# CFSAN-Biostatistics/snp-pipeline

Hardware: AMD Instinct MI355X
Metric: consensus_bases_called_per_sec (higher is better)
Workload: dtype u8; 1 GPU; BASELINE configs[3] shard (125 samples/GPU x 5000000 bp x 30x synthetic pileups, 49878 SNP sites, 1500 SNP records per sample; the reference bundles no pileups); step = site-record gather + site union, one batched scan launch + one call launch, 4-bit pack, row all-gather, all-pairs distance tiles, row-band exchange; samples_total=125, samples_this_rank=125, genome_bp=5000000, snp_sites=49878, pileup_bytes_this_rank=54061520755, parallelism=samples sharded over 1 rank(s)

## Files before the change

### include/snpgpu.h

```cpp
#ifndef SNPGPU_H
#define SNPGPU_H

#include <stddef.h>
#include <stdint.h>

#ifdef __cplusplus
extern "C" {
#endif

#define SNPGPU_ABI_VERSION 7

#define SNPGPU_OK            0
#define SNPGPU_E_HIP        -1
#define SNPGPU_E_ARG        -2
#define SNPGPU_E_NOMEM      -3
#define SNPGPU_E_PILEUP     -4
#define SNPGPU_E_UNSUPPORTED -5
#define SNPGPU_E_IO         -6
#define SNPGPU_E_TIMEOUT    -7

#define SNPGPU_F_RAWDPTH  0x01
#define SNPGPU_F_VARFREQ  0x02
#define SNPGPU_F_DEPTH    0x04
#define SNPGPU_F_STRDPTH  0x08
// ... 282 lines not shown
uint32_t snpgpu_symbol_spill_capacity(const snpgpu_ctx *ctx);

typedef struct snpgpu_consensus_job {
    const char *fasta_path;
    const char *fasta_id;
    const uint8_t *sequence;
    uint64_t n_bases;
    const char *vcf_path;
    const char *vcf_header;
    const snpgpu_site_counts *counts;
    const uint64_t *line_off;
    const uint8_t *row_filters;
    const uint8_t *site_in_flow;
    int32_t rc;
    uint32_t n_rows;
} snpgpu_consensus_job;
int  snpgpu_write_consensus_files(snpgpu_consensus_job *jobs, uint32_t n_jobs, uint32_t n_sites, const uint8_t *contig_names,
                                  const uint32_t *contig_name_off, const uint64_t *site_keys, const char *const *filter_names,
                                  int preserve_ref_case, char failed_snp_gt, const snpgpu_symbol_spill *spill, uint32_t n_spill,
                                  uint32_t n_threads);

int  snpgpu_region_flow_dev(snpgpu_ctx *ctx, const uint8_t *d_base, const uint8_t *d_filters, const uint64_t *d_line_off,
                            uint32_t n_samples, uint32_t n_sites, const uint32_t *d_cols, const int32_t *d_col_of, uint32_t n_cols,
                            const uint32_t *d_excl_off, const uint32_t *d_excl_slots, uint8_t *d_out_base, uint8_t *d_out_filters,
                            uint32_t *d_err);

int  snpgpu_rows_copy_dev(snpgpu_ctx *ctx, const void *d_src, uint64_t src_stride, const uint32_t *d_src_index,
                          void *d_dst, uint64_t dst_stride, const uint32_t *d_dst_index, uint32_t n_rows, uint64_t row_bytes);

int  snpgpu_siteset_line_offsets(snpgpu_ctx *ctx, const snpgpu_siteset *ss, uint64_t *out_line_off);

#define SNPGPU_CALL_PASSES 4
int  snpgpu_call_pass_counts(snpgpu_ctx *ctx, uint64_t out[SNPGPU_CALL_PASSES]);

size_t snpgpu_packed_row_bytes(uint32_t n_sites);
int  snpgpu_pack_matrix_dev(snpgpu_ctx *ctx, const uint8_t *d_symbols, uint32_t n_rows, uint32_t n_sites,
                            size_t row_stride, void *d_packed);
int  snpgpu_distance_packed_dev(snpgpu_ctx *ctx, const void *d_packed, uint32_t n_rows, uint32_t n_sites,
                                uint32_t tile_rank, uint32_t tile_nranks, int32_t *d_out);
int  snpgpu_distance(snpgpu_ctx *ctx, const uint8_t *symbols, uint32_t n_rows, uint32_t n_sites, int32_t *out);

int  snpgpu_vcf_sites(const char *path, uint64_t capacity, uint32_t *out_pos, uint32_t *out_contig, uint64_t *out_n_records,
                      char *out_names, uint64_t names_capacity, uint64_t *out_name_off, uint32_t names_max,
                      uint32_t *out_n_names);
int  snpgpu_snplist_sites(const char *path, uint64_t capacity, uint32_t *out_pos, uint32_t *out_contig, uint64_t *out_n_records,
                          char *out_names, uint64_t names_capacity, uint64_t *out_name_off, uint32_t names_max,
                          uint32_t *out_n_names);
int  snpgpu_write_snplist(const char *path, const char *contig_names, const uint64_t *contig_off, const uint64_t *keys,
                          uint64_t n_sites, const uint32_t *carrier_off, const uint32_t *carriers, const char *sample_names,
                          const uint64_t *sample_off);

int  snpgpu_fasta_scan(const char *path, uint64_t *out_n_records, uint64_t *out_max_len, uint64_t *out_names_bytes);
int  snpgpu_fasta_load(const char *path, uint64_t n_records, uint64_t row_stride, uint8_t pad, uint8_t *out_matrix,
                       uint64_t *out_len, char *out_names, uint64_t *out_name_off);

#define SNPGPU_TSV_PAIRWISE 0
#define SNPGPU_TSV_MATRIX   1
int  snpgpu_write_distance_tsv(const char *path, int layout, const char *ids, const uint64_t *id_off, uint32_t n,
                               const int32_t *matrix, uint64_t row_stride);

#define SNPGPU_COMM_ID_BYTES 128
int  snpgpu_comm_available(void);
int  snpgpu_comm_version(int *out_version);
int  snpgpu_comm_unique_id(void *out_id);
int  snpgpu_comm_init(snpgpu_ctx *ctx, int rank, int nranks, const void *unique_id);
void snpgpu_comm_destroy(snpgpu_ctx *ctx);
// ... 108 lines not shown
```

### snp_pipeline_amd/_lib.py

```python
import ctypes as C
import os

_HERE = os.path.dirname(os.path.abspath(__file__))
LIB_PATH = os.path.join(_HERE, "lib", "libsnpgpu.so")

MAX_SYMS = 8
SCAN_STATUS_WORDS = 4
CALL_PASSES = 4

F_RAWDPTH, F_VARFREQ, F_DEPTH, F_STRDPTH, F_STRBIAS, F_REGION = 1, 2, 4, 8, 16, 32
SITE_IN_SNPLIST, SITE_EXCLUDED = 1, 2
ST_NO_LINE, ST_OK, ST_SHORT_LINE, ST_BAD_DEPTH, ST_NO_QUALS, ST_MULTI_REF = 0, 1, 2, 3, 4, 5
VCF_LINE_WINDOW, VCF_MORE_UNUSUAL, VCF_LONG_LINE = 4096, 1, 2
E_HIP, E_ARG, E_NOMEM, E_PILEUP, E_UNSUPPORTED, E_IO, E_TIMEOUT = -1, -2, -3, -4, -5, -6, -7


class CallerParams(C.Structure):
    _fields_ = [("min_base_quality", C.c_int32), ("min_cons_depth", C.c_int32),
                ("min_cons_strand_depth", C.c_int32), ("reserved", C.c_int32),
                ("min_cons_freq", C.c_double), ("min_cons_strand_bias", C.c_double)]


class SiteCounts(C.Structure):
    _fields_ = [("raw_depth", C.c_uint32), ("good_depth", C.c_uint32), ("fwd_good_depth", C.c_uint32),
# ... 121 lines not shown
    "snpgpu_call_consensus_batch_dev": (C.c_int, [_P, _P, _P, _P, _P, C.c_uint32, C.POINTER(CallerParams), _P, _P, _P]),
    "snpgpu_call_consensus": (C.c_int, [_P, _P, _P, C.c_size_t, C.POINTER(CallerParams), _P, _P, _P, _P, C.c_int]),
    "snpgpu_call_consensus_files": (C.c_int, [_P, _P, C.POINTER(C.c_char_p), C.c_uint32, C.POINTER(CallerParams), _P, _P, _P, _P,
                                              _P, _P, _P, _P, C.POINTER(StreamOpts), C.POINTER(StreamStats)]),
    "snpgpu_call_consensus_files_dev": (C.c_int, [_P, _P, C.POINTER(C.c_char_p), C.c_uint32, C.POINTER(CallerParams), _P, _P, _P, _P,
                                                  _P, _P, _P, _P, C.POINTER(StreamOpts), C.POINTER(StreamStats)]),
    "snpgpu_call_consensus_many_dev": (C.c_int, [_P, _P, _P, _P, C.c_uint32, C.POINTER(CallerParams), _P, _P, _P, _P, _P, _P, C.c_int]),
    "snpgpu_region_flow_dev": (C.c_int, [_P, _P, _P, _P, C.c_uint32, C.c_uint32, _P, _P, C.c_uint32, _P, _P, _P, _P, _P]),
    "snpgpu_rows_copy_dev": (C.c_int, [_P, _P, C.c_uint64, _P, _P, C.c_uint64, _P, C.c_uint32, C.c_uint64]),
    "snpgpu_write_consensus_files": (C.c_int, [_P, C.c_uint32, C.c_uint32, _P, _P, _P, C.POINTER(C.c_char_p), C.c_int, C.c_char, _P, C.c_uint32,
                                               C.c_uint32]),
    "snpgpu_varscan_dev": (C.c_int, [_P, _P, C.c_uint64, _P, C.c_uint32, _P, C.POINTER(C.c_uint32), _P]),
    "snpgpu_varscan_batch_dev": (C.c_int, [_P, _P, _P, C.c_uint32, _P, C.c_uint32, _P, _P, _P, _P]),
    "snpgpu_pileups_create": (C.c_int, [_P, C.c_uint64, C.POINTER(_P)]),
    "snpgpu_pileups_destroy": (None, [_P]),
    "snpgpu_pileups_ingest": (C.c_int, [_P, _P, C.POINTER(C.c_char_p), C.c_uint32, _P, C.c_uint32, _P, _P, _P, _P, _P]),
    "snpgpu_pileups_count": (C.c_uint32, [_P]),
    "snpgpu_pileups_get": (C.c_int, [_P, C.c_uint32, C.POINTER(_P), C.POINTER(C.c_uint64)]),
    "snpgpu_pileups_get_stats": (C.c_int, [_P, C.POINTER(PileupsStats)]),
    "snpgpu_call_all_lines_file": (C.c_int, [_P, _P, C.c_char_p, C.POINTER(CallerParams), C.c_uint64, C.POINTER(C.c_uint64),
                                             _P, _P, _P, _P]),
    "snpgpu_call_all_lines_compact_file": (C.c_int, [_P, _P, C.c_char_p, C.POINTER(CallerParams), C.c_uint64, C.POINTER(C.c_uint64), _P, _P,
                                                     C.c_uint32, C.POINTER(C.c_uint32), _P, _P, _P]),
    "snpgpu_format_line_rows": (C.c_size_t, [_P, C.c_uint64, _P, _P, C.c_uint64, _P, _P, C.c_uint32, C.POINTER(C.c_char_p), C.c_int, C.c_char, _P, C.c_uint32,
                                             C.c_int, _P, C.c_size_t, C.POINTER(C.c_uint64), C.POINTER(C.c_int64)]),
    "snpgpu_write_all_positions_vcf": (C.c_int, [_P, _P, C.c_char_p, C.POINTER(CallerParams), C.c_char_p, C.c_char_p, C.POINTER(C.c_char_p), C.c_int, C.c_char,
                                                 C.c_int, C.c_int, C.POINTER(C.c_uint64), C.POINTER(C.c_uint64), C.POINTER(C.c_uint64), C.POINTER(C.c_uint64), _P, _P]),
    "snpgpu_format_vcf_rows": (C.c_size_t, [_P, _P, C.c_uint32, _P, _P, _P, C.POINTER(C.c_char_p), C.c_int, C.c_char, _P, C.c_uint32, _P,
                                            C.c_size_t, C.POINTER(C.c_int32)]),
    "snpgpu_symbol_spill_read": (C.c_int, [_P, _P, C.c_uint32, C.POINTER(C.c_uint32)]),
    "snpgpu_symbol_spill_capacity": (C.c_uint32, [_P]),
    "snpgpu_siteset_line_offsets": (C.c_int, [_P, _P, _P]),
    "snpgpu_call_pass_counts": (C.c_int, [_P, _P]),
    "snpgpu_packed_row_bytes": (C.c_size_t, [C.c_uint32]),
    "snpgpu_pack_matrix_dev": (C.c_int, [_P, _P, C.c_uint32, C.c_uint32, C.c_size_t, _P]),
    "snpgpu_distance_packed_dev": (C.c_int, [_P, _P, C.c_uint32, C.c_uint32, C.c_uint32, C.c_uint32, _P]),
    "snpgpu_distance": (C.c_int, [_P, _P, C.c_uint32, C.c_uint32, _P]),
    "snpgpu_varscan_file": (C.c_int, [_P, C.c_char_p, _P, C.c_uint32, _P, C.POINTER(C.c_uint32), _P]),
    "snpgpu_varscan_files": (C.c_int, [_P, C.POINTER(C.c_char_p), C.c_uint32, _P, C.c_uint32, _P, _P, _P, _P]),
    "snpgpu_varscan_format_rows": (C.c_size_t, [_P, C.c_uint32, _P, C.c_uint64, _P, _P, C.c_size_t, C.POINTER(C.c_uint32)]),
    "snpgpu_vcf_count_snps_file": (C.c_int, [_P, C.c_char_p, C.c_uint32, _P, _P, _P]),
    "snpgpu_vcf_count_snps_files": (C.c_int, [_P, C.POINTER(C.c_char_p), C.c_uint32, C.c_uint32, _P, _P, _P, _P]),
    "snpgpu_fasta_scan": (C.c_int, [C.c_char_p, C.POINTER(C.c_uint64), C.POINTER(C.c_uint64), C.POINTER(C.c_uint64)]),
    "snpgpu_fasta_load": (C.c_int, [C.c_char_p, C.c_uint64, C.c_uint64, C.c_uint8, _P, _P, _P, _P]),
    "snpgpu_vcf_sites": (C.c_int, [C.c_char_p, C.c_uint64, _P, _P, C.POINTER(C.c_uint64), _P, C.c_uint64, _P, C.c_uint32, C.POINTER(C.c_uint32)]),
    "snpgpu_snplist_sites": (C.c_int, [C.c_char_p, C.c_uint64, _P, _P, C.POINTER(C.c_uint64), _P, C.c_uint64, _P, C.c_uint32, C.POINTER(C.c_uint32)]),
    "snpgpu_write_snplist": (C.c_int, [C.c_char_p, _P, _P, _P, C.c_uint64, _P, _P, _P, _P]),
    "snpgpu_write_distance_tsv": (C.c_int, [C.c_char_p, C.c_int, _P, _P, C.c_uint32, _P, C.c_uint64]),
    "snpgpu_dense_windows": (C.c_int, [_P, _P, _P, C.c_uint32, _P, _P, C.c_uint32, _P, _P, _P, C.POINTER(C.c_uint32)]),
    "snpgpu_merge_regions": (C.c_int, [_P, _P, _P, _P, C.c_uint32, _P, _P, _P, C.POINTER(C.c_uint32)]),
    "snpgpu_in_regions": (C.c_int, [_P, _P, _P, C.c_uint32, _P, _P, _P, C.c_uint32, _P]),
    "snpgpu_merge_sites": (C.c_int, [_P, _P, _P, C.c_size_t, _P, _P, _P, C.POINTER(C.c_uint32), C.POINTER(C.c_uint32)]),
    "snpgpu_dense_windows_dev": (C.c_int, [_P, _P, _P, C.c_uint32, C.c_uint32, _P, _P, C.c_uint32, _P, _P, _P, _P]),
    "snpgpu_merge_regions_dev": (C.c_int, [_P, _P, _P, _P, C.c_uint32, _P, _P, _P, _P]),
    "snpgpu_in_regions_dev": (C.c_int, [_P, _P, _P, C.c_uint32, _P, _P, _P, C.c_uint32, _P]),
    "snpgpu_merge_vcf_files": (C.c_int, [_P, C.POINTER(C.c_char_p), C.c_uint32, C.c_char_p, C.c_char_p, C.c_uint32, C.c_uint32, _P]),
    "snpgpu_merge_vcf_files_opts": (C.c_int, [_P, C.POINTER(C.c_char_p), C.c_uint32, C.c_char_p, C.c_char_p, C.c_uint32, _P, _P, _P]),
    "snpgpu_merge_plan": (C.c_int, [C.c_uint32, C.c_uint64, C.c_uint64, _P, _P]),
    "snpgpu_merge_sites_dev": (C.c_int, [_P, _P, _P, C.c_uint32, _P, _P, _P, _P]),
    "snpgpu_comm_available": (C.c_int, []),
    "snpgpu_comm_version": (C.c_int, [C.POINTER(C.c_int)]),
    "snpgpu_comm_unique_id": (C.c_int, [_P]),
    "snpgpu_comm_init": (C.c_int, [_P, C.c_int, C.c_int, _P]),
    "snpgpu_comm_destroy": (None, [_P]),
    "snpgpu_comm_abort": (None, [_P]),
    "snpgpu_comm_info": (C.c_int, [_P, C.POINTER(C.c_int), C.POINTER(C.c_int), C.POINTER(C.c_int)]),
# ... 53 lines not shown
```

### snp_pipeline_amd/csrc/consensus.hip

```cpp
#include <stdlib.h>

#include "internal.h"

#define CALL_WAVES 4
#define CALL_LBUF 4224
#define CALL_LMAX 2048
#define HIST_BINS 384

struct CallArgs {
    const SampleDev *samples;
    uint32_t n_samples;
    const uint64_t *site_line;
    const uint8_t *site_flags;
    uint32_t flags_stride;
    uint32_t n_sites;
    snpgpu_caller_params prm;
    uint8_t *out_base;
    uint8_t *out_filters;
    snpgpu_site_counts *out_counts;
    uint64_t *todo;
    uint32_t *todo_n;
    const uint64_t *in_todo;
    const uint32_t *in_todo_n;
    const uint32_t *deep;
    snpgpu_symbol_spill *spill;
    uint32_t *spill_n;
    uint32_t spill_cap;
};

struct WaveLds {
    uint8_t line[CALL_LBUF];
    uint8_t s1[CALL_LMAX + 64];
    uint32_t hist[HIST_BINS];
    uint32_t fs[6], fe[6];
// ... 378 lines not shown
template <int N> __device__ __forceinline__ BM<N> m_bit(uint32_t i) { BM<N> r; BM_FOR r.w[k_] = (i >> 6) == (uint32_t)k_ ? 1ull << (i & 63u) : 0ull; return r; }
template <int N> __device__ __forceinline__ uint64_t m_word(BM<N> a, uint32_t idx) { uint64_t r = a.w[0]; BM_FOR if (idx == (uint32_t)k_) r = a.w[k_]; return r; }
template <int N> __device__ __forceinline__ bool m_test(BM<N> a, uint32_t i) { return ((m_word(a, (i >> 6) & (N - 1)) >> (i & 63u)) & 1ull) != 0; }
template <int N> __device__ __forceinline__ uint32_t m_ctz(BM<N> a) {
    uint32_t r = 64u * N;
#pragma unroll
    for (int k = N - 1; k >= 0; --k) if (a.w[k]) r = 64u * k + (uint32_t)__builtin_ctzll(a.w[k]);
    return r;
}
template <int N> __device__ __forceinline__ uint32_t m_popc(BM<N> a) { uint32_t r = 0; BM_FOR r += (uint32_t)__popcll(a.w[k_]); return r; }
template <int N> __device__ __forceinline__ BM<N> m_clear_lowest(BM<N> a) {
    bool done = false;
    BM_FOR if (!done && a.w[k_]) { a.w[k_] &= a.w[k_] - 1; done = true; }
    return a;
}

struct Planes {
    uint32_t p0, p1, p2, p3, p4, p5, p6;
    __device__ __forceinline__ uint32_t punct() const { return ~p6 & p5 & ~p4; }
    __device__ __forceinline__ uint32_t caret() const { return p6 & ~p5 & p4 & p3 & p2 & p1 & ~p0; }
    __device__ __forceinline__ uint32_t sign() const { return punct() & p3 & p0 & (p2 ^ p1); }
    __device__ __forceinline__ uint32_t dollar() const { return punct() & ~p3 & p2 & ~p1 & ~p0; }
    __device__ __forceinline__ uint32_t digit() const { return ~p6 & p5 & p4 & ~(p3 & (p2 | p1)); }
    struct Symbols { uint32_t a5, c5, g5, n5, t5, star, dot, comma; };
    __device__ __forceinline__ Symbols symbols(uint32_t keep) const {
        const uint32_t lo3 = ~p4 & ~p3, ac = lo3 & ~p2 & p0;
        const uint32_t kp = keep & ~p6 & p5 & ~p4 & p3 & ~p0;
        return Symbols{ac & ~p1, ac & p1, lo3 & p2 & p1 & p0, ~p4 & p3 & p2 & p1 & ~p0, p4 & ~p3 & p2 & ~p1 & ~p0, kp & ~p2 & p1, kp & p2 & p1, kp & p2 & ~p1};
    }
    __device__ __forceinline__ uint32_t upper() const { return p6 & ~p5; }
    __device__ __forceinline__ uint32_t lower() const { return p6 & p5; }
};

template <int kWin, int kWaves>
struct LanesLds {
    uint32_t slot[kWaves][64 * (kWin / 4 + 1)];
    uint8_t cls[256];
    uint4 hist[kWaves][64];
};

template <int kWin, int kWords, int kWaves, bool kCounts>
__global__ __launch_bounds__(kWaves * 64, kWin == 128 ? 3 : 1) void k_call_lanes(CallArgs a) {
    constexpr int LANES_WIN = kWin;
    constexpr int LANES_STRIDE = kWin / 4 + 1;
    constexpr int LANES_WAVES = kWaves;
    constexpr uint32_t kBits = 64u * kWords;
    constexpr uint32_t kMaxField = kBits > 255u ? 255u : kBits;
    typedef BM<kWords> M;
    __shared__ LanesLds<kWin, kWaves> S;
    const bool deep = a.deep && *a.deep != 0;
    if (kWin == 128 && deep) return;
    if (kWin == 256 && deep) { a.in_todo = nullptr; a.in_todo_n = nullptr; }
    for (uint32_t c = threadIdx.x; c < 256; c += blockDim.x) {
        const uint32_t u = to_upper(c);
        uint32_t k = u == '*' ? 0u : u == 'A' ? 1u : u == 'C' ? 2u : u == 'G' ? 3u : u == 'N' ? 4u : u == 'T' ? 5u : 0xFFu;
        if (k != 0xFFu && c >= 0x61u) k |= 8u;
        if (c == '.') k = 6u;
        if (c == ',') k = 14u;
        S.cls[c] = (uint8_t)k;
    }
    __syncthreads();
    const uint32_t lane = lane_id();
    const uint32_t wave = __builtin_amdgcn_readfirstlane(threadIdx.x >> 6);
    uint32_t *slot = &S.slot[wave][lane * LANES_STRIDE];
    const uint8_t *slot_b = (const uint8_t *)slot;
    const uint64_t n_work = a.in_todo ? (uint64_t)*a.in_todo_n : (uint64_t)a.n_samples * a.n_sites;
    const uint64_t n_groups = (n_work + 63) / 64;
    const int minq = a.prm.min_base_quality;

    struct LaneRef { uint64_t site; uint64_t lv; uint32_t sflags; uintptr_t buf, end; };
    auto fetch_ref = [&](uint64_t g) -> LaneRef {
        LaneRef r{0, 0, 0, 0, 0};
        const uint64_t idx = g * 64 + lane;
        if (g < n_groups && idx < n_work) {
            const uint64_t s = a.in_todo ? a.in_todo[idx] : idx;
            const uint32_t sample = (uint32_t)(s / a.n_sites);
            r.site = s;
            r.lv = a.site_line[s];
            r.sflags = a.site_flags[s - (uint64_t)sample * a.n_sites + (uint64_t)sample * a.flags_stride];
            r.buf = (uintptr_t)a.samples[sample].buf;
            r.end = r.buf + a.samples[sample].nbytes;
        }
        return r;
    };
    const uint64_t g_stride = (uint64_t)gridDim.x * LANES_WAVES;
    uint64_t grp = (uint64_t)blockIdx.x * LANES_WAVES + wave;
    LaneRef nxt = fetch_ref(grp);
    for (; grp < n_groups; grp += g_stride) {
        const LaneRef cur = nxt;
        nxt = fetch_ref(grp + g_stride);
        const uint64_t site = cur.site;
        const bool valid = grp * 64 + lane < n_work;
        const uint64_t lv = cur.lv;
        const uint32_t sflags = cur.sflags;
        const uintptr_t addr = cur.buf + (lv - 1), end = cur.end;
        const bool has = lv != 0;
#if defined(SNPGPU_TUNING) && defined(CALL_EXP_ALIGN128)
        const uintptr_t al = addr & ~(uintptr_t)127;
#else
        const uintptr_t al = addr & ~(uintptr_t)15;
#endif
        const uint32_t o = (uint32_t)(addr & 15);
        auto stage_half = [&](int half, bool want) {
            if (!__ballot(want && end - al < (uintptr_t)LANES_WIN + 16)) {
                const uint64_t wm = __ballot(want);
                const uint32_t piece = lane & 7u;
                uint4 v[8];
#pragma unroll
                for (int r = 0; r < 8; ++r) {
                    const uint32_t src = 8u * r + (lane >> 3);
                    const uint32_t lo = (uint32_t)__builtin_amdgcn_ds_bpermute((int)(src << 2), (int)(uint32_t)al);
                    const uint32_t hi = (uint32_t)__builtin_amdgcn_ds_bpermute((int)(src << 2), (int)(uint32_t)(al >> 32));
                    const uintptr_t x = (((uintptr_t)hi << 32) | lo) + 128u * half + 16u * piece;
                    v[r] = make_uint4(0, 0, 0, 0);
                    if ((wm >> src) & 1ull) v[r] = *(const uint4 *)x;
                }
#pragma unroll
                for (int r = 0; r < 8; ++r) {
                    const uint32_t src = 8u * r + (lane >> 3);
                    if ((wm >> src) & 1ull) {
                        uint32_t *dst = &S.slot[wave][src * LANES_STRIDE + 32 * half + 4 * piece];
                        dst[0] = v[r].x; dst[1] = v[r].y; dst[2] = v[r].z; dst[3] = v[r].w;
                    }
                }
                return;
            }
            uint4 v[8];
#pragma unroll
            for (int r = 0; r < 8; ++r) {
                const uintptr_t x = al + 16u * (8 * half + r);
                v[r] = make_uint4(0x0A0A0A0Au, 0x0A0A0A0Au, 0x0A0A0A0Au, 0x0A0A0A0Au);
                if (want && x < end) v[r] = *(const uint4 *)x;
            }
#pragma unroll
            for (int r = 0; r < 8; ++r) {
                const uintptr_t x = al + 16u * (8 * half + r);
                if (__ballot(want && x < end && x + 16 > end)) {
                    uint32_t w[4] = {v[r].x, v[r].y, v[r].z, v[r].w};
#pragma unroll
                    for (int d = 0; d < 4; ++d)
#pragma unroll
                        for (int bb = 0; bb < 4; ++bb)
                            if (x + 4 * d + bb >= end) w[d] = (w[d] & ~(0xFFu << (8 * bb))) | (0x0Au << (8 * bb));
                    v[r] = make_uint4(w[0], w[1], w[2], w[3]);
                }
                if (want) {
                    uint32_t *dst = slot + 4 * (8 * half + r);
                    dst[0] = v[r].x; dst[1] = v[r].y; dst[2] = v[r].z; dst[3] = v[r].w;
                }
            }
        };
        stage_half(0, has);
        __builtin_amdgcn_wave_barrier();
#if defined(SNPGPU_TUNING) && defined(CALL_EXP) && CALL_EXP >= 2
// ... 7 lines not shown
        bool done = !has;
#pragma unroll
        for (int blk = 0; blk < LANES_WIN / 64; ++blk) {
            if (!__ballot(!done)) break;
            if (blk >= 2 && (blk & 1) == 0) { stage_half(blk / 2, !done); __builtin_amdgcn_wave_barrier(); }
            const bool open = !done;
            uint32_t mw[2] = {0, 0}, mt[2] = {0, 0};
#pragma unroll
            for (int jp = 0; jp < 8; ++jp) {
                uint32_t w2[2] = {slot[16 * blk + 2 * jp], slot[16 * blk + 2 * jp + 1]};
                if (blk == 0 && jp < 2) {
#pragma unroll
                    for (int h = 0; h < 2; ++h) {
                        const uint32_t j = 2 * jp + h;
                        const uint32_t nb = o > 4u * j ? min(o - 4u * j, 4u) : 0u;
                        const uint32_t m = nb >= 4 ? 0xFFFFFFFFu : ((1u << (8 * nb)) - 1u);
                        w2[h] = (w2[h] & ~m) | (0x20202020u & m);
                    }
                }
                const uint64_t W = (uint64_t)w2[0] | ((uint64_t)w2[1] << 32);
                const uint64_t ge9 = W + 0x7777777777777777ull, ge14 = W + 0x7272727272727272ull, ge10 = W + 0x7676767676767676ull;
                const uint64_t ge28 = W + 0x6464646464646464ull, ge33 = W + 0x5F5F5F5F5F5F5F5Full;
                const uint64_t f_ws = ((ge9 & ~ge14) | (ge28 & ~ge33)) & 0x8080808080808080ull;
                const uint64_t f_t = ge10 & ~ge14 & 0x8080808080808080ull;
                const uint32_t bw = __builtin_amdgcn_udot4((uint32_t)(f_ws >> 32), 0x80402010u, __builtin_amdgcn_udot4((uint32_t)f_ws, 0x08040201u, 0u, false), false) >> 7;
                const uint32_t bt = __builtin_amdgcn_udot4((uint32_t)(f_t >> 32), 0x80402010u, __builtin_amdgcn_udot4((uint32_t)f_t, 0x08040201u, 0u, false), false) >> 7;
                mw[jp >> 2] |= bw << (8 * (jp & 3));
                mt[jp >> 2] |= bt << (8 * (jp & 3));
            }
            Wm[blk] = open ? (uint64_t)mw[0] | ((uint64_t)mw[1] << 32) : ~0ull;
            Tm[blk] = open ? (uint64_t)mt[0] | ((uint64_t)mt[1] << 32) : 0ull;
            done = done || Tm[blk] != 0;
        }
        auto scan_from = [&](const uint64_t (&Mk)[LANES_WIN / 64], bool inv, uint32_t pos) -> uint32_t {
            uint32_t r = LANES_WIN;
#pragma unroll
            for (int j = LANES_WIN / 64 - 1; j >= 0; --j) {
                uint64_t m = inv ? ~Mk[j] : Mk[j];
                const uint32_t pj = pos >> 6;
                m = pj > (uint32_t)j ? 0ull : (pj == (uint32_t)j ? m & (~0ull << (pos & 63u)) : m);
                if (m) r = 64u * j + (uint32_t)__builtin_ctzll(m);
            }
            return r;
        };
        const uint32_t line_end = scan_from(Tm, false, 0);
        uint32_t nf = 0, f_s[6], f_e[6];
        {
            uint32_t pos = o;
#pragma unroll
            for (int k = 0; k < 6; ++k) {
                const uint32_t st = scan_from(Wm, true, pos);
                const uint32_t en = scan_from(Wm, false, st < (uint32_t)LANES_WIN ? st : LANES_WIN - 1u);
                const bool found = st < line_end;
                nf += found ? 1u : 0u;
                f_s[k] = st; f_e[k] = en;
                pos = found ? (en < (uint32_t)LANES_WIN ? en : LANES_WIN - 1u) : LANES_WIN - 1u;
            }
        }
        bool punt = has && line_end >= (uint32_t)LANES_WIN;
        if (has && !punt) { const uint32_t tc = slot_b[line_end]; punt = tc == 11u || tc == 12u; }
        auto fs = [&](int k) -> uint32_t { return f_s[k]; };
        auto fe = [&](int k) -> uint32_t { return f_e[k]; };
        uint32_t ref = 0, raw_depth = 0;
        if (has && !punt) {
            if (nf < 4 || nf == 5 || fe(2) - fs(2) != 1 || fe(3) - fs(3) > 9 || fe(3) <= fs(3)) punt = true;
            else {
                ref = slot_b[fs(2)];
                for (uint32_t q = fs(3); q < fe(3); ++q) {
                    const uint32_t c = slot_b[q];
                    if (!is_digit(c)) punt = true;
                    raw_depth = raw_depth * 10u + (c - 48u);
                }
            }
        }
        uint64_t cnt_f = 0, cnt_r = 0;
        uint32_t good = 0;
        bool parse = has && !punt && raw_depth != 0 && nf >= 6;
        if (parse && fe(4) - fs(4) > kMaxField) { punt = true; parse = false; }
        {
            const uint32_t bs = parse ? fs(4) : 0u, L0 = parse ? fe(4) - fs(4) : 0u, qs = fs(5), qlen = parse ? fe(5) - fs(5) : 0u;
            uint32_t maxL = L0;
            for (int off = 32; off; off >>= 1) maxL = max(maxL, (uint32_t)__shfl_xor((int)maxL, off));
            maxL = __builtin_amdgcn_readfirstlane(maxL);
            const uint32_t nd = (maxL + 3) >> 2;
            const M V = m_below<kWords>(L0);
            uint32_t pl[7][2 * kWords];
#pragma unroll
            for (int b = 0; b < 7; ++b)
#pragma unroll
                for (int q = 0; q < 2 * kWords; ++q) pl[b][q] = 0;
            {
                const uint32_t sh = bs & 3u;
                uint32_t lo = slot[bs >> 2];
#pragma unroll
                for (uint32_t jp = 0; jp < 8u * kWords; ++jp) {
// ... 230 lines not shown
                rec[6] = make_uint4(tr[0], tr[1], tr[2], tr[3]); rec[7] = make_uint4(tr[4], tr[5], tr[6], tr[7]);
            }
        }
        const uint64_t pm = __ballot(punt);
        if (pm) {
            uint32_t base = 0;
            if (lane == 0) base = atomicAdd(a.todo_n, (uint32_t)__popcll(pm));
            base = __builtin_amdgcn_readfirstlane(base);
            if (punt) a.todo[base + __popcll(pm & low_mask(lane))] = site;
        }
        __builtin_amdgcn_wave_barrier();
    }
}

__global__ __launch_bounds__(256) void k_call_mode(const SampleDev *samples, uint32_t n, uint32_t *deep, uint64_t all_lines) {
    __shared__ unsigned long long part[3][4];
    unsigned long long bytes = 0, lines = 0, hits = 0;
    for (uint32_t i = threadIdx.x; i < n; i += blockDim.x) { bytes += samples[i].nbytes; lines += samples[i].status[1]; hits += samples[i].status[2]; }
    for (int o = 32; o; o >>= 1) { bytes += __shfl_xor(bytes, o); lines += __shfl_xor(lines, o); hits += __shfl_xor(hits, o); }
    if ((threadIdx.x & 63) == 0) { part[0][threadIdx.x >> 6] = bytes; part[1][threadIdx.x >> 6] = lines; part[2][threadIdx.x >> 6] = hits; }
    __syncthreads();
    if (threadIdx.x == 0) {
        bytes = part[0][0] + part[0][1] + part[0][2] + part[0][3];
        lines = part[1][0] + part[1][1] + part[1][2] + part[1][3];
        hits = all_lines ? all_lines : part[2][0] + part[2][1] + part[2][2] + part[2][3];
        *deep = bytes > 100ull * lines ? 1u : 0u;
        deep[1] = (uint32_t)hits;
        deep[2] = (uint32_t)(hits >> 32);
    }
}

struct SampleIO { const uint8_t *d_pileup; size_t nbytes; uint64_t *d_status; };

static int enqueue_call_n(snpgpu_ctx *ctx, uint32_t n_sites, const uint8_t *default_flags, const SampleDev *d_table, uint32_t n,
                          const snpgpu_caller_params *prm, const uint64_t *d_site_line, uint8_t *d_out_base,
                          uint8_t *d_out_filters, snpgpu_site_counts *d_out_counts, uint32_t *d_todo_n, uint64_t *d_todo,
                          uint64_t *d_todo2, const uint8_t *d_site_flags, uint32_t flags_stride, bool all_lines = false) {
    hipStream_t st = ctx->stream;
    if (!n_sites || !n) return SNPGPU_OK;
    ctx->call_passes_from = d_todo_n == ctx->d_call_ctl ? 1 : 0;
    CallArgs ca;
    ca.samples = d_table;
    ca.n_samples = n;
    ca.site_line = d_site_line;
    ca.site_flags = d_site_flags ? d_site_flags : default_flags;
    ca.flags_stride = d_site_flags ? flags_stride : 0;
    ca.n_sites = n_sites;
    ca.prm = *prm;
    ca.out_base = d_out_base;
    ca.out_filters = d_out_filters;
    ca.out_counts = d_out_counts;
    ca.spill = d_out_counts ? ctx->d_spill : nullptr;
    ca.spill_n = ctx->d_spill_n;
    ca.spill_cap = ctx->spill_cap;
    const uint64_t n_work = (uint64_t)n_sites * n;
    const uint64_t blocks = (n_work + CALL_WAVES - 1) / CALL_WAVES;
    const uint64_t max_blocks = (uint64_t)ctx->n_cu * 16;
    const unsigned grid = (unsigned)(blocks < max_blocks ? blocks : max_blocks);
    ca.todo = nullptr;
    ca.todo_n = nullptr;
    ca.in_todo = nullptr;
    ca.in_todo_n = nullptr;
    ca.deep = nullptr;
    hipEvent_t ta = snpgpu_time_begin(ctx);
    {
        const uint64_t groups = (n_work + 63) / 64;
        k_call_mode<<<1, 256, 0, st>>>(d_table, n, d_todo_n + SNPGPU_CALL_CTL_MODE, all_lines ? (uint64_t)n_sites : 0ull);
        ca.deep = d_todo_n + SNPGPU_CALL_CTL_MODE;
        ca.todo = d_todo;
        ca.todo_n = d_todo_n;
        const uint64_t b0 = (groups + 3) / 4, m0 = (uint64_t)ctx->n_cu * 16;
        const unsigned g0 = (unsigned)(b0 < m0 ? b0 : m0);
        if (d_out_counts) k_call_lanes<128, 1, 4, true><<<g0, 256, 0, st>>>(ca); else k_call_lanes<128, 1, 4, false><<<g0, 256, 0, st>>>(ca);
        ca.in_todo = d_todo;
        ca.in_todo_n = d_todo_n;
        ca.todo = d_todo2;
        ca.todo_n = d_todo_n + 1;
        const uint64_t lblocks = (groups + 1) / 2, lmax = (uint64_t)ctx->n_cu * 8;
        const unsigned g1 = (unsigned)(lblocks < lmax ? lblocks : lmax);
        if (d_out_counts) k_call_lanes<256, 2, 2, true><<<g1, 128, 0, st>>>(ca); else k_call_lanes<256, 2, 2, false><<<g1, 128, 0, st>>>(ca);
        ca.in_todo = d_todo2;
        ca.in_todo_n = d_todo_n + 1;
        ca.todo = d_todo;
        ca.todo_n = d_todo_n + 2;
        const uint64_t l2max = (uint64_t)ctx->n_cu * 4;
        const unsigned g2 = (unsigned)(groups < l2max ? groups : l2max);
        if (d_out_counts) k_call_lanes<512, 4, 1, true><<<g2, 64, 0, st>>>(ca); else k_call_lanes<512, 4, 1, false><<<g2, 64, 0, st>>>(ca);
        k_call_sites<<<grid, CALL_WAVES * 64, 0, st>>>(ca);
    }
    snpgpu_time_end(ctx, SNPGPU_K_CALL, ta);
    HIP_TRY(ctx, hipGetLastError());
    return SNPGPU_OK;
}

int snpgpu_enqueue_call(snpgpu_ctx *ctx, const snpgpu_siteset *ss, const SampleDev *d_table, uint32_t n,
                        const snpgpu_caller_params *prm, const uint64_t *d_site_line, uint8_t *d_out_base,
                        uint8_t *d_out_filters, snpgpu_site_counts *d_out_counts, uint32_t *d_todo_n, uint64_t *d_todo,
                        uint64_t *d_todo2, const uint8_t *d_site_flags, uint32_t flags_stride) {
    return enqueue_call_n(ctx, ss->n_sites, ss->dev.flags, d_table, n, prm, d_site_line, d_out_base, d_out_filters, d_out_counts, d_todo_n, d_todo, d_todo2,
                          d_site_flags, flags_stride);
}

int snpgpu_enqueue_call_lines(snpgpu_ctx *ctx, const SampleDev *d_sample, const uint64_t *d_line_off, const uint8_t *d_flags,
                              uint32_t n_lines, const snpgpu_caller_params *prm, uint8_t *d_out_base, uint8_t *d_out_filters,
// ... 49 lines not shown
    uint64_t *d_todo2 = (uint64_t *)((char *)ws + ws_bytes + rows_bytes + list_bytes);
    std::vector<SampleDev> samples(n);
    for (uint32_t i = 0; i < n; ++i) {
        samples[i] = SampleDev{};
        samples[i].buf = io[i].d_pileup;
        samples[i].nbytes = io[i].nbytes;
        samples[i].status = io[i].d_status;
    }
    int rc = snpgpu_enqueue_scan(ctx, ss, samples, ws, d_site_line, want_depth, d_todo_n, SNPGPU_CALL_PASSES - 1);
    if (rc) return rc;
    return snpgpu_enqueue_call(ctx, ss, (const SampleDev *)ws, n, prm, d_site_line, d_out_base, d_out_filters, d_out_counts,
                               d_todo_n, d_todo, d_todo2, d_site_flags, flags_stride);
}

static int enqueue_sample(snpgpu_ctx *ctx, const snpgpu_siteset *ss, const uint8_t *d_pileup, size_t nbytes,
                          const snpgpu_caller_params *prm, uint8_t *d_out_base, uint8_t *d_out_filters,
                          snpgpu_site_counts *d_out_counts, uint64_t *d_status, int want_depth) {
    SampleIO io{d_pileup, nbytes, d_status};
    return enqueue_group(ctx, ss, &io, 1, prm, d_out_base, d_out_filters, d_out_counts, ss->site_line, want_depth);
}

uint32_t *snpgpu_call_ctl(snpgpu_ctx *ctx) {
    if (!ctx->d_call_ctl) {
        void *d = nullptr;
        if (hipMalloc(&d, 256) != hipSuccess) { snpgpu_set_error(ctx, SNPGPU_E_HIP, "hipMalloc of the call chain's counters failed"); return nullptr; }
        if (hipMemsetAsync(d, 0, 256, ctx->stream) != hipSuccess) { (void)hipFree(d); snpgpu_set_error(ctx, SNPGPU_E_HIP, "hipMemsetAsync failed"); return nullptr; }
        ctx->d_call_ctl = (uint32_t *)d;
    }
    return ctx->d_call_ctl;
}

extern "C" {

int snpgpu_call_pass_counts(snpgpu_ctx *ctx, uint64_t out[SNPGPU_CALL_PASSES]) {
    if (!ctx || !out) return snpgpu_set_error(ctx, SNPGPU_E_ARG, "null argument");
    for (int k = 0; k < SNPGPU_CALL_PASSES; ++k) out[k] = 0;
    if (ctx->call_passes_from == 2) { out[SNPGPU_CALL_PASSES - 1] = ctx->call_passes_all; return SNPGPU_OK; }
    if (ctx->call_passes_from != 1 || !ctx->d_call_ctl) return SNPGPU_OK;
    HIP_TRY(ctx, snpgpu_enter(ctx));
    uint32_t h[SNPGPU_CALL_CTL_WORDS];
    HIP_TRY(ctx, hipMemcpyAsync(h, ctx->d_call_ctl, sizeof h, hipMemcpyDeviceToHost, ctx->stream));
    HIP_TRY(ctx, hipStreamSynchronize(ctx->stream));
    const uint64_t with_line = (uint64_t)h[SNPGPU_CALL_CTL_MODE + 1] | ((uint64_t)h[SNPGPU_CALL_CTL_MODE + 2] << 32);
    const int first = h[SNPGPU_CALL_CTL_MODE] ? 1 : 0;
    uint64_t before = with_line;
    for (int k = first; k < SNPGPU_CALL_PASSES - 1; ++k) {
        out[k] = before > h[k] ? before - h[k] : 0;
        before = h[k];
    }
    out[SNPGPU_CALL_PASSES - 1] = before;
    return SNPGPU_OK;
}

int snpgpu_call_consensus_dev(snpgpu_ctx *ctx, const snpgpu_siteset *ss, const void *d_pileup, size_t nbytes,
                              const snpgpu_caller_params *params, uint8_t *d_out_base, uint8_t *d_out_filters,
                              snpgpu_site_counts *d_out_counts, uint64_t *d_status, int want_depth_sum) {
    if (!ctx || !ss || !params || !d_status || (nbytes && !d_pileup)) return snpgpu_set_error(ctx, SNPGPU_E_ARG, "null argument");
    if (ss->n_sites && (!d_out_base || !d_out_filters)) return snpgpu_set_error(ctx, SNPGPU_E_ARG, "null output");
    HIP_TRY(ctx, snpgpu_enter(ctx));
    if (d_out_counts) { int rc = snpgpu_spill_begin(ctx); if (rc) return rc; }
    return enqueue_sample(ctx, ss, (const uint8_t *)d_pileup, nbytes, params, d_out_base, d_out_filters, d_out_counts, d_status, want_depth_sum);
}

int snpgpu_siteset_line_offsets(snpgpu_ctx *ctx, const snpgpu_siteset *ss, uint64_t *out_line_off) {
    if (!ctx || !ss || (ss->n_sites && !out_line_off)) return snpgpu_set_error(ctx, SNPGPU_E_ARG, "null argument");
    if (!ss->n_sites) return SNPGPU_OK;
// ... 66 lines not shown
```

### snp_pipeline_amd/csrc/internal.h

```cpp
#pragma once

#include <hip/hip_runtime.h>
#include <stdint.h>
#include <stdio.h>
#include <string>
#include <vector>

#include "../../include/snpgpu.h"
#include "bgzf_host.h"

struct snpgpu_stream_pool;
void snpgpu_stream_pool_destroy(struct snpgpu_ctx *ctx);
void snpgpu_comm_release(struct snpgpu_ctx *ctx);

struct snpgpu_ctx {
    int device = 0;
    snpgpu_stream_pool *pool = nullptr;
    hipStream_t stream = nullptr;
    hipStream_t own_stream = nullptr;
    hipEvent_t ev_start = nullptr, ev_stop = nullptr;
    std::string err;
    void *scratch = nullptr;
    size_t scratch_bytes = 0;
    int n_cu = 256;
    bool scan_lds_attr = false;
    bool varscan_lds_attr = false;
    bool bgzf_lds_attr = false;
    void *comm = nullptr;
    snpgpu_symbol_spill *d_spill = nullptr;
    uint32_t *d_spill_n = nullptr;
    uint32_t *d_call_ctl = nullptr;
    int call_passes_from = 0;
    uint64_t call_passes_all = 0;
    uint32_t spill_cap = 0, spill_want = SNPGPU_SPILL_CAP;
    bool time_kernels = false;
    struct Timed { int kernel; hipEvent_t a, b; };
    std::vector<Timed> timed;
    std::vector<hipEvent_t> event_pool;
};

#define SNPGPU_SLOW_QUEUE_CAP (1u << 20)
#define SNPGPU_K_SCAN 0
#define SNPGPU_K_CALL 1
#define SNPGPU_K_DISTANCE 2
#define SNPGPU_K_VARSCAN 3
#define SNPGPU_K_VCF_COUNT 4
#define SNPGPU_K_VCF_MERGE 5
#define SNPGPU_K_BGZF 6
int snpgpu_spill_begin(snpgpu_ctx *ctx);
hipEvent_t snpgpu_time_begin(snpgpu_ctx *ctx);
void snpgpu_time_end(snpgpu_ctx *ctx, int kernel, hipEvent_t a);

struct snpgpu_pileups {
    snpgpu_ctx *ctx = nullptr;
    uint64_t budget = 0;
    uint64_t used = 0;
    std::vector<void *> blocks;
    struct Entry { uint8_t *d = nullptr; uint64_t nbytes = 0; bool resident = false; };
    std::vector<Entry> files;
    uint64_t h2d_bytes = 0;
    uint64_t file_bytes = 0;
    double seconds = 0, seconds_allocating = 0, seconds_waiting_for_readers = 0, seconds_waiting_for_device = 0;
    double reader_seconds_reading = 0, reader_seconds_waiting = 0, seconds_preparing = 0;
    uint32_t n_readers = 0;
};
// ... 186 lines not shown
```

### snp_pipeline_amd/device.py

```python
import ctypes as C
import os

import numpy as np

from . import _lib as L
from ._lib import CallerParams, SiteCounts, SnpGpuError

COUNTS_DTYPE = np.dtype([
    ("raw_depth", "<u4"), ("good_depth", "<u4"), ("fwd_good_depth", "<u4"), ("rev_good_depth", "<u4"),
    ("n_symbols", "<u4"), ("ref_base", "u1"), ("cons_base", "u1"), ("filters", "u1"), ("status", "u1"),
    ("sym", "u1", (L.MAX_SYMS,)), ("total", "<u4", (L.MAX_SYMS,)), ("fwd", "<u4", (L.MAX_SYMS,)),
    ("rev", "<u4", (L.MAX_SYMS,))])
assert COUNTS_DTYPE.itemsize == 128
LINE_WIDE, LINE_SYMS = 0xFF, 3
LINE_DTYPE = np.dtype([("raw_depth", "<u4"), ("total", "<u2", (LINE_SYMS,)), ("fwd", "<u2", (LINE_SYMS,)), ("rev", "<u2", (LINE_SYMS,)),
                       ("sym", "u1", (LINE_SYMS,)), ("ref_base", "u1"), ("cons_base", "u1"), ("filters", "u1"), ("status", "u1"),
                       ("n_symbols", "u1"), ("site_flags", "u1"), ("reserved", "u1")])
assert LINE_DTYPE.itemsize == 32
VARSCAN_DTYPE = np.dtype([("line_off", "<u8"), ("sdp", "<u4"), ("dp", "<u4"), ("total", "<u4"), ("rdf", "<u4"), ("rdr", "<u4"),
                          ("ref_qual_sum", "<u4"), ("adf", "<u4"), ("adr", "<u4"), ("alt_qual_sum", "<u4"), ("ref_base", "u1"),
                          ("alt_base", "u1"), ("reserved", "u1", (2,))])
assert VARSCAN_DTYPE.itemsize == 48

_SCAN_CODES = {1: "line has fewer than 2 fields", 2: "position field is not an unsigned decimal integer",
# ... 684 lines not shown
            if err is not None:
                raise err

    def raise_file_errors(self, siteset, path, params, rc, res, wanted=None):
        repeats = res.line_offsets is not None and res.n_matched > int(np.count_nonzero(res.line_offsets))
        if not repeats or rc == L.E_IO:
            self.raise_file_status(path, rc, res, True, wanted)
            return
        self.call_all_lines(siteset, path, params, capacity=res.n_lines, check=True, listed_only=True)
        if rc != 0 and rc not in (L.E_PILEUP, L.E_UNSUPPORTED):
            raise SnpGpuError(int(rc), "pileup %s" % path)

    def check_repeated_positions(self, siteset, path, params, res):
        if res.line_offsets is None or res.n_matched <= int(np.count_nonzero(res.line_offsets)):
            return
        _, flags, counts = self.call_all_lines(siteset, path, params, capacity=res.n_lines, check=False)
        bad = np.nonzero((flags != 0) & (counts["status"] > L.ST_OK))[0]
        if len(bad):
            err, _ = self.site_error(ConsensusResult(None, None, counts[bad[:1]], res.status))
            raise err

    def line_offsets(self, siteset):
        out = np.zeros(len(siteset), dtype=np.uint64)
        self._check(self.lib.snpgpu_siteset_line_offsets(self.ctx, siteset.handle, _ptr(out)))
        return out

    CALL_PASS_NAMES = ("lanes128", "lanes256", "lanes512", "wave")

    def call_pass_counts(self):
        out = np.zeros(L.CALL_PASSES, dtype=np.uint64)
        self._check(self.lib.snpgpu_call_pass_counts(self.ctx, _ptr(out)))
        return dict(zip(self.CALL_PASS_NAMES, (int(v) for v in out)))

    def call_consensus_dev(self, siteset, d_pileup_ptr, nbytes, params, d_bases, d_filters, d_status, d_counts=None,
                           want_depth_sum=False):
        self._check(self.lib.snpgpu_call_consensus_dev(
            self.ctx, siteset.handle, C.c_void_p(d_pileup_ptr), nbytes, C.byref(params), C.c_void_p(d_bases),
            C.c_void_p(d_filters), C.c_void_p(d_counts) if d_counts else None, C.c_void_p(d_status),
            1 if want_depth_sum else 0))

    def call_consensus_batch_dev(self, siteset, d_pileups_ptr, offsets, params, d_bases, d_filters, d_status, sizes=None):
        offs = np.ascontiguousarray(offsets, dtype=np.uint64)
        if sizes is None:
            n, sz = len(offs) - 1, None
        else:
            sz = np.ascontiguousarray(sizes, dtype=np.uint64)
            n = len(sz)
            if len(offs) < n:
                raise ValueError("offsets shorter than sizes")
        self._check(self.lib.snpgpu_call_consensus_batch_dev(
            self.ctx, siteset.handle, C.c_void_p(d_pileups_ptr), _ptr(offs), _ptr(sz) if sz is not None else None, n,
            C.byref(params), C.c_void_p(d_bases), C.c_void_p(d_filters), C.c_void_p(d_status)))

    def call_consensus_many_dev(self, siteset, d_ptrs, sizes, params, d_bases, d_filters, d_status, d_counts=0, d_line_off=0,
                                d_site_flags=0, want_depth_sum=False):
        n = len(sizes)
        ptrs = (C.c_void_p * max(n, 1))(*[C.c_void_p(int(p)) for p in d_ptrs])
        sz = np.ascontiguousarray(sizes, dtype=np.uint64)
        opt = lambda v: C.c_void_p(v) if v else None
        self._check(self.lib.snpgpu_call_consensus_many_dev(
            self.ctx, siteset.handle, ptrs, _ptr(sz), n, C.byref(params), opt(d_site_flags), C.c_void_p(d_bases), C.c_void_p(d_filters),
            opt(d_counts), opt(d_line_off), C.c_void_p(d_status), 1 if want_depth_sum else 0))

    def region_flow_dev(self, d_base, d_filters, d_line_off, n_samples, n_sites, d_cols, d_col_of, n_cols, d_excl_off, d_excl_slots,
                        d_out_base, d_out_filters, d_err):
        opt = lambda v: C.c_void_p(v) if v else None
# ... 383 lines not shown
```

Before: 706.7 million bases/s.

## Rework lanes128 call kernel field parsing, staging, prefetch and grid sizing

Replaces the serial six-field scan in the 128-byte lanes call kernel with a bitmask-based field extractor that finds field boundaries from edge masks using popcount and clear-lowest operations. It also simplifies the LDS staging addressing in bpermute pulls and drops the next-group prefetch for the 128 window to save registers. The launch grid is now sized from queried occupancy (blocks per CU) times a fixed round count instead of a fixed 16 blocks per CU. This aims to cut scalar scan work and register pressure, but the new field extractor only tracks fields two through five and relies on the caller's punt checks for correctness.

```diff
diff --git a/include/snpgpu.h b/include/snpgpu.h
--- a/include/snpgpu.h
+++ b/include/snpgpu.h
@@ -338,6 +338,7 @@
 
 #define SNPGPU_CALL_PASSES 4
 int  snpgpu_call_pass_counts(snpgpu_ctx *ctx, uint64_t out[SNPGPU_CALL_PASSES]);
+int  snpgpu_call_lanes128_resident(snpgpu_ctx *ctx, uint32_t *workgroups);
 
 size_t snpgpu_packed_row_bytes(uint32_t n_sites);
 int  snpgpu_pack_matrix_dev(snpgpu_ctx *ctx, const uint8_t *d_symbols, uint32_t n_rows, uint32_t n_sites,
diff --git a/snp_pipeline_amd/_lib.py b/snp_pipeline_amd/_lib.py
--- a/snp_pipeline_amd/_lib.py
+++ b/snp_pipeline_amd/_lib.py
@@ -177,6 +177,7 @@
     "snpgpu_symbol_spill_capacity": (C.c_uint32, [_P]),
     "snpgpu_siteset_line_offsets": (C.c_int, [_P, _P, _P]),
     "snpgpu_call_pass_counts": (C.c_int, [_P, _P]),
+    "snpgpu_call_lanes128_resident": (C.c_int, [_P, C.POINTER(C.c_uint32)]),
     "snpgpu_packed_row_bytes": (C.c_size_t, [C.c_uint32]),
     "snpgpu_pack_matrix_dev": (C.c_int, [_P, _P, C.c_uint32, C.c_uint32, C.c_size_t, _P]),
     "snpgpu_distance_packed_dev": (C.c_int, [_P, _P, C.c_uint32, C.c_uint32, C.c_uint32, C.c_uint32, _P]),
diff --git a/snp_pipeline_amd/csrc/call_fields.h b/snp_pipeline_amd/csrc/call_fields.h
--- /dev/null
+++ b/snp_pipeline_amd/csrc/call_fields.h
@@ -0,0 +1,82 @@
+#pragma once
+#include <stdint.h>
+#ifndef __HIP_DEVICE_COMPILE__
+#include <assert.h>
+#endif
+
+#if defined(__HIPCC__) || defined(__CUDACC__)
+#define CALL_FIELDS_FN __host__ __device__ inline
+#else
+#define CALL_FIELDS_FN inline
+#endif
+
+struct CallFields {
+    uint32_t line_end;
+    uint32_t nf;
+    uint32_t s[4], e[4];
+};
+
+CALL_FIELDS_FN uint32_t cf_ffbl(uint32_t d) {
+#ifdef __HIP_DEVICE_COMPILE__
+    uint32_t f;
+    asm("v_ffbl_b32 %0, %1" : "=v"(f) : "v"(d));
+    return f;
+#else
+    return d ? (uint32_t)__builtin_ctz(d) : ~0u;
+#endif
+}
+
+template <int N> CALL_FIELDS_FN uint32_t cf_ctz(const uint64_t (&x)[N]) {
+    uint32_t r = 64u * N;
+#pragma unroll
+    for (int h = 0; h < 2 * N; ++h) {
+        const uint32_t f = cf_ffbl((uint32_t)(x[h >> 1] >> (32 * (h & 1)))) | (32u * h);
+        r = f < r ? f : r;
+    }
+    return r;
+}
+
+template <int N> CALL_FIELDS_FN void cf_clear_lowest(uint64_t (&x)[N]) {
+    static_assert(N % 2 == 0, "pairs of words");
+    typedef unsigned __int128 u128;
+    bool borrow = true;
+#pragma unroll
+    for (int k = 0; k < N; k += 2) {
+        const u128 v = (u128)x[k] | ((u128)x[k + 1] << 64);
+        const u128 r = v & (v - (borrow ? 1u : 0u));
+        x[k] = (uint64_t)r;
+        x[k + 1] = (uint64_t)(r >> 64);
+        borrow = borrow && v == 0;
+    }
+}
+
+template <int N> CALL_FIELDS_FN CallFields call_fields(const uint64_t (&Wm)[N], const uint64_t (&Tm)[N], uint32_t o) {
+#ifndef __HIP_DEVICE_COMPILE__
+    assert(o < 64u && (Wm[0] & ((1ull << o) - 1)) == (1ull << o) - 1 && (Tm[0] & ((1ull << o) - 1)) == 0);
+#endif
+    (void)o;
+    CallFields f;
+    f.line_end = cf_ctz<N>(Tm);
+    uint64_t X[N];
+    bool below_empty = true;
+    uint32_t n = 0;
+#pragma unroll
+    for (int k = 0; k < N; ++k) {
+        const uint64_t upto = below_empty ? Tm[k] ^ (Tm[k] - 1) : 0ull;
+        below_empty = below_empty && Tm[k] == 0;
+        X[k] = (Wm[k] ^ ((Wm[k] << 1) | (k ? Wm[k ? k - 1 : 0] >> 63 : 1ull))) & upto;
+        n += (uint32_t)__builtin_popcountll(X[k]);
+    }
+    const uint32_t runs = (n + 1) >> 1;
+    f.nf = runs < 6u ? runs : 6u;
+#pragma unroll
+    for (int k = 0; k < 4; ++k) cf_clear_lowest<N>(X);
+#pragma unroll
+    for (int k = 0; k < 4; ++k) {
+        f.s[k] = cf_ctz<N>(X);
+        cf_clear_lowest<N>(X);
+        f.e[k] = cf_ctz<N>(X);
+        if (k < 3) cf_clear_lowest<N>(X);
+    }
+    return f;
+}
diff --git a/snp_pipeline_amd/csrc/consensus.hip b/snp_pipeline_amd/csrc/consensus.hip
--- a/snp_pipeline_amd/csrc/consensus.hip
+++ b/snp_pipeline_amd/csrc/consensus.hip
@@ -1,5 +1,6 @@
 #include <stdlib.h>
 
+#include "call_fields.h"
 #include "internal.h"
 
 #define CALL_WAVES 4
@@ -444,6 +445,10 @@
     __device__ __forceinline__ uint32_t lower() const { return p6 & p5; }
 };
 
+#ifndef CALL_LANES128_PER_SIMD
+#define CALL_LANES128_PER_SIMD 3
+#endif
+#define CALL_LANES128_ROUNDS 4
 template <int kWin, int kWaves>
 struct LanesLds {
     uint32_t slot[kWaves][64 * (kWin / 4 + 1)];
@@ -452,7 +457,7 @@
 };
 
 template <int kWin, int kWords, int kWaves, bool kCounts>
-__global__ __launch_bounds__(kWaves * 64, kWin == 128 ? 3 : 1) void k_call_lanes(CallArgs a) {
+__global__ __launch_bounds__(kWaves * 64, kWin == 128 ? CALL_LANES128_PER_SIMD : 1) void k_call_lanes(CallArgs a) {
     constexpr int LANES_WIN = kWin;
     constexpr int LANES_STRIDE = kWin / 4 + 1;
     constexpr int LANES_WAVES = kWaves;
@@ -497,10 +502,12 @@
     };
     const uint64_t g_stride = (uint64_t)gridDim.x * LANES_WAVES;
     uint64_t grp = (uint64_t)blockIdx.x * LANES_WAVES + wave;
-    LaneRef nxt = fetch_ref(grp);
+    constexpr bool kFetchEarly = kWin != 128;
+    LaneRef nxt{0, 0, 0, 0, 0};
+    if (kFetchEarly) nxt = fetch_ref(grp);
     for (; grp < n_groups; grp += g_stride) {
-        const LaneRef cur = nxt;
-        nxt = fetch_ref(grp + g_stride);
+        const LaneRef cur = kFetchEarly ? nxt : fetch_ref(grp);
+        if (kFetchEarly) nxt = fetch_ref(grp + g_stride);
         const uint64_t site = cur.site;
         const bool valid = grp * 64 + lane < n_work;
         const uint64_t lv = cur.lv;
@@ -515,23 +522,25 @@
         const uint32_t o = (uint32_t)(addr & 15);
         auto stage_half = [&](int half, bool want) {
             if (!__ballot(want && end - al < (uintptr_t)LANES_WIN + 16)) {
-                const uint64_t wm = __ballot(want);
+                uint32_t row = lane >> 3;
+                asm volatile("" : "+v"(row));
+                const uint64_t wl = __ballot(want) >> row;
                 const uint32_t piece = lane & 7u;
+                const uint32_t pull = row << 2;
+                uint32_t *dst0 = &S.slot[wave][row * LANES_STRIDE + 32 * half + 4 * piece];
                 uint4 v[8];
 #pragma unroll
                 for (int r = 0; r < 8; ++r) {
-                    const uint32_t src = 8u * r + (lane >> 3);
-                    const uint32_t lo = (uint32_t)__builtin_amdgcn_ds_bpermute((int)(src << 2), (int)(uint32_t)al);
-                    const uint32_t hi = (uint32_t)__builtin_amdgcn_ds_bpermute((int)(src << 2), (int)(uint32_t)(al >> 32));
+                    const uint32_t lo = (uint32_t)__builtin_amdgcn_ds_bpermute((int)(pull + 32u * r), (int)(uint32_t)al);
+                    const uint32_t hi = (uint32_t)__builtin_amdgcn_ds_bpermute((int)(pull + 32u * r), (int)(uint32_t)(al >> 32));
                     const uintptr_t x = (((uintptr_t)hi << 32) | lo) + 128u * half + 16u * piece;
                     v[r] = make_uint4(0, 0, 0, 0);
-                    if ((wm >> src) & 1ull) v[r] = *(const uint4 *)x;
+                    if ((wl >> (8 * r)) & 1ull) v[r] = *(const uint4 *)x;
                 }
 #pragma unroll
                 for (int r = 0; r < 8; ++r) {
-                    const uint32_t src = 8u * r + (lane >> 3);
-                    if ((wm >> src) & 1ull) {
-                        uint32_t *dst = &S.slot[wave][src * LANES_STRIDE + 32 * half + 4 * piece];
+                    if ((wl >> (8 * r)) & 1ull) {
+                        uint32_t *dst = dst0 + 8 * r * LANES_STRIDE;
                         dst[0] = v[r].x; dst[1] = v[r].y; dst[2] = v[r].z; dst[3] = v[r].w;
                     }
                 }
@@ -605,35 +614,12 @@
             Tm[blk] = open ? (uint64_t)mt[0] | ((uint64_t)mt[1] << 32) : 0ull;
             done = done || Tm[blk] != 0;
         }
-        auto scan_from = [&](const uint64_t (&Mk)[LANES_WIN / 64], bool inv, uint32_t pos) -> uint32_t {
-            uint32_t r = LANES_WIN;
-#pragma unroll
-            for (int j = LANES_WIN / 64 - 1; j >= 0; --j) {
-                uint64_t m = inv ? ~Mk[j] : Mk[j];
-                const uint32_t pj = pos >> 6;
-                m = pj > (uint32_t)j ? 0ull : (pj == (uint32_t)j ? m & (~0ull << (pos & 63u)) : m);
-                if (m) r = 64u * j + (uint32_t)__builtin_ctzll(m);
-            }
-            return r;
-        };
-        const uint32_t line_end = scan_from(Tm, false, 0);
-        uint32_t nf = 0, f_s[6], f_e[6];
-        {
-            uint32_t pos = o;
-#pragma unroll
-            for (int k = 0; k < 6; ++k) {
-                const uint32_t st = scan_from(Wm, true, pos);
-                const uint32_t en = scan_from(Wm, false, st < (uint32_t)LANES_WIN ? st : LANES_WIN - 1u);
-                const bool found = st < line_end;
-                nf += found ? 1u : 0u;
-                f_s[k] = st; f_e[k] = en;
-                pos = found ? (en < (uint32_t)LANES_WIN ? en : LANES_WIN - 1u) : LANES_WIN - 1u;
-            }
-        }
+        const CallFields fld = call_fields<LANES_WIN / 64>(Wm, Tm, o);
+        const uint32_t line_end = fld.line_end, nf = fld.nf;
         bool punt = has && line_end >= (uint32_t)LANES_WIN;
         if (has && !punt) { const uint32_t tc = slot_b[line_end]; punt = tc == 11u || tc == 12u; }
-        auto fs = [&](int k) -> uint32_t { return f_s[k]; };
-        auto fe = [&](int k) -> uint32_t { return f_e[k]; };
+        auto fs = [&](int k) -> uint32_t { return fld.s[k - 2]; };
+        auto fe = [&](int k) -> uint32_t { return fld.e[k - 2]; };
         uint32_t ref = 0, raw_depth = 0;
         if (has && !punt) {
             if (nf < 4 || nf == 5 || fe(2) - fs(2) != 1 || fe(3) - fs(3) > 9 || fe(3) <= fs(3)) punt = true;
@@ -930,6 +916,16 @@
 
 struct SampleIO { const uint8_t *d_pileup; size_t nbytes; uint64_t *d_status; };
 
+static int lanes128_per_cu(snpgpu_ctx *ctx) {
+    if (ctx->call_lanes128_per_cu) return SNPGPU_OK;
+    int with = 0, without = 0;
+    HIP_TRY(ctx, hipOccupancyMaxActiveBlocksPerMultiprocessor(&with, (k_call_lanes<128, 1, 4, true>), 256, 0));
+    HIP_TRY(ctx, hipOccupancyMaxActiveBlocksPerMultiprocessor(&without, (k_call_lanes<128, 1, 4, false>), 256, 0));
+    if (with < 1 || without < 1) return snpgpu_set_error(ctx, SNPGPU_E_HIP, "k_call_lanes<128> does not fit on a compute unit");
+    ctx->call_lanes128_per_cu = with < without ? with : without;
+    return SNPGPU_OK;
+}
+
 static int enqueue_call_n(snpgpu_ctx *ctx, uint32_t n_sites, const uint8_t *default_flags, const SampleDev *d_table, uint32_t n,
                           const snpgpu_caller_params *prm, const uint64_t *d_site_line, uint8_t *d_out_base,
                           uint8_t *d_out_filters, snpgpu_site_counts *d_out_counts, uint32_t *d_todo_n, uint64_t *d_todo,
@@ -960,6 +956,7 @@
     ca.in_todo = nullptr;
     ca.in_todo_n = nullptr;
     ca.deep = nullptr;
+    { int rc = lanes128_per_cu(ctx); if (rc) return rc; }
     hipEvent_t ta = snpgpu_time_begin(ctx);
     {
         const uint64_t groups = (n_work + 63) / 64;
@@ -967,7 +964,11 @@
         ca.deep = d_todo_n + SNPGPU_CALL_CTL_MODE;
         ca.todo = d_todo;
         ca.todo_n = d_todo_n;
-        const uint64_t b0 = (groups + 3) / 4, m0 = (uint64_t)ctx->n_cu * 16;
+        uint64_t rounds = CALL_LANES128_ROUNDS;
+#ifdef SNPGPU_TUNING
+        if (const char *e = getenv("SNPGPU_CALL_ROUNDS")) if (atoi(e) > 0) rounds = (uint64_t)atoi(e);
+#endif
+        const uint64_t b0 = (groups + 3) / 4, m0 = (uint64_t)ctx->n_cu * ctx->call_lanes128_per_cu * rounds;
         const unsigned g0 = (unsigned)(b0 < m0 ? b0 : m0);
         if (d_out_counts) k_call_lanes<128, 1, 4, true><<<g0, 256, 0, st>>>(ca); else k_call_lanes<128, 1, 4, false><<<g0, 256, 0, st>>>(ca);
         ca.in_todo = d_todo;
@@ -1083,6 +1084,14 @@
 
 extern "C" {
 
+int snpgpu_call_lanes128_resident(snpgpu_ctx *ctx, uint32_t *workgroups) {
+    if (!ctx || !workgroups) return snpgpu_set_error(ctx, SNPGPU_E_ARG, "null argument");
+    int rc = lanes128_per_cu(ctx);
+    if (rc) return rc;
+    *workgroups = (uint32_t)ctx->n_cu * (uint32_t)ctx->call_lanes128_per_cu;
+    return SNPGPU_OK;
+}
+
 int snpgpu_call_pass_counts(snpgpu_ctx *ctx, uint64_t out[SNPGPU_CALL_PASSES]) {
     if (!ctx || !out) return snpgpu_set_error(ctx, SNPGPU_E_ARG, "null argument");
     for (int k = 0; k < SNPGPU_CALL_PASSES; ++k) out[k] = 0;
diff --git a/snp_pipeline_amd/csrc/internal.h b/snp_pipeline_amd/csrc/internal.h
--- a/snp_pipeline_amd/csrc/internal.h
+++ b/snp_pipeline_amd/csrc/internal.h
@@ -31,6 +31,7 @@
     uint32_t *d_spill_n = nullptr;
     uint32_t *d_call_ctl = nullptr;
     int call_passes_from = 0;
+    int call_lanes128_per_cu = 0;
     uint64_t call_passes_all = 0;
     uint32_t spill_cap = 0, spill_want = SNPGPU_SPILL_CAP;
     bool time_kernels = false;
diff --git a/snp_pipeline_amd/device.py b/snp_pipeline_amd/device.py
--- a/snp_pipeline_amd/device.py
+++ b/snp_pipeline_amd/device.py
@@ -740,6 +740,11 @@
         self._check(self.lib.snpgpu_call_pass_counts(self.ctx, _ptr(out)))
         return dict(zip(self.CALL_PASS_NAMES, (int(v) for v in out)))
 
+    def call_lanes128_resident(self):
+        n = C.c_uint32()
+        self._check(self.lib.snpgpu_call_lanes128_resident(self.ctx, C.byref(n)))
+        return int(n.value)
+
     def call_consensus_dev(self, siteset, d_pileup_ptr, nbytes, params, d_bases, d_filters, d_status, d_counts=None,
                            want_depth_sum=False):
         self._check(self.lib.snpgpu_call_consensus_dev(
```

Result: no change. 710.3 million bases/s (median of 6 runs) (+0.5%).
